# aatifjiwani/lens-flare

Measured on AMD Instinct MI355X. Metric: Mray-surface-intersections/s + frame time, 1080p 256spp double-Gauss, higher is better.
Workload: dtype f32

## Files before the change

lens-flare_amd/csrc/lf_cull_prepass.hip:

```cpp
#include <algorithm>
#include <chrono>
#include <cmath>
#include <cstdio>
#include <cstdlib>
#include <cstring>

#include "lf_internal.h"
#include "lf_march_events.h"
#include "lf_march_common.h"

namespace {

using namespace lfm;

constexpr int kCullSamples = 15;
struct CullLevelArgs {
  int W, H;
  float pitch, half_w, half_h;
  int blocks_x, blocks_y, blk_log2;
  int share_rank, share_n, share_nb;
  int P;
  int P_final;
  int last;
  int n_paths;
// ... 394 lines not shown
__device__ __forceinline__ float ship_extent(const ShipFoot& f, float geo_margin, float nx, float ny) {
  const float e = fabsf(fmaf(f.g1x, nx, f.g1y * ny)) + fabsf(fmaf(f.g2x, nx, f.g2y * ny)) +
                  fabsf(fmaf(f.gxx, nx, f.gxy * ny)) + fabsf(fmaf(f.gyx, nx, f.gyy * ny));
  return fminf(f.ball, fmaf(geo_margin, e, f.slack));
}
__device__ __forceinline__ bool ship_lobe_culls(const ShipFoot& f, float geo_margin, float sx, float sy, float rho) {
  const float ex = sx - f.cx, ey = sy - f.cy;
  const float dist = lf_sqrt(fmaf(ex, ex, ey * ey));
  const float id = dist > 0.0f ? lf_rcp(dist) : 0.0f;
  return dist - kShipLobeK * ship_extent(f, geo_margin, ex * id, ey * id) > rho;
}

template <class A>
__device__ __forceinline__ unsigned ship_lobes_reached(const ShipFoot& f, float geo_margin, unsigned live, const A& a) {
  for (int k = 0; k < a.n_lights; k++)
    if (((live >> k) & 1u) != 0u && ship_lobe_culls(f, geo_margin, a.lsx[k], a.lsy[k], a.lrho[k])) live &= ~(1u << k);
  return live;
}

constexpr unsigned kSlotCulled = 0u, kSlotKept = 1u, kSlotFoot = 2u;
constexpr int kCullMaxLevels = 8;
struct CullCacheOut {
  unsigned* slots;
  float4* foots;
  unsigned* foot_count;
  unsigned foot_cap;
  unsigned n_mine;
};

template <bool BUILD, bool LIGHTS = false>
__device__ __forceinline__ void cull_level_body(const LfLensDev* __restrict__ lens,
                                                    const LfPairsDev* __restrict__ pairs,
                                                    const int* __restrict__ seq_table,
                                                    const LfProgRow* __restrict__ rec_table, const CullLevelArgs& a,
                                                    const unsigned* __restrict__ items,
                                                    const unsigned* __restrict__ counts, unsigned items_stride,
                                                    unsigned* __restrict__ next, unsigned* __restrict__ next_counts,
                                                    unsigned long long* __restrict__ table,
                                                    unsigned long long* __restrict__ stats, const CullCacheOut& co) {
  const int q = blockIdx.y;
  const unsigned PP = (unsigned)(a.P * a.P);
  const unsigned n_blk = (unsigned)(a.blocks_x * a.blocks_y);
  const unsigned n_mine = (n_blk + (unsigned)a.share_n - 1u - (unsigned)a.share_rank) / (unsigned)a.share_n;
  const unsigned n_items = items ? min(counts[q], items_stride) : n_mine * PP;
  const unsigned i = blockIdx.x * blockDim.x + threadIdx.x;
  if ((i & ~63u) >= n_items) return;
  const bool valid = i < n_items;
  const unsigned item = valid ? (items ? items[(size_t)q * items_stride + i]
                                       : ((unsigned)a.share_rank + (unsigned)a.share_n * (i / PP)) * PP + i % PP) : 0u;
  const int blk = (int)(item / PP), cell = (int)(item % PP);
  const int ci = cell % a.P, cj = cell / a.P;
  const int bx = blk % a.blocks_x, by = blk / a.blocks_x;

  const float px0 = (float)(bx << a.blk_log2), px1 = fminf((float)a.W, (float)((bx + 1) << a.blk_log2));
  const float py0 = (float)(by << a.blk_log2), py1 = fminf((float)a.H, (float)((by + 1) << a.blk_log2));
  const float Xc = -((0.5f * (px0 + px1)) - a.half_w) * a.pitch, Yc = -((0.5f * (py0 + py1)) - a.half_h) * a.pitch;
  const float hX = 0.5f * (px1 - px0) * a.pitch, hY = 0.5f * (py1 - py0) * a.pitch;
  const float invP = 1.0f / (float)a.P;

  const int n_ev = pairs->ev_cnt[q];
  const int* const seq = seq_table + pairs->ev_off[q];
  const int lane = (int)(threadIdx.x & 63u);
  constexpr unsigned kAll = (1u << kCullSamples) - 1u;
  const LfProgRow* recs_of[3];
  int j_of[3];
  float ns_of[3];
#pragma unroll
  for (int w = 0; w < 3; w++) {
    const int l = a.lam[w], g = l / a.march_k;
    j_of[w] = l - g * a.march_k;
    recs_of[w] = rec_table + (size_t)g * (size_t)a.prog_recs;
    ns_of[w] = lens->n_start[l];
  }
  Ray r[kCullSamples];
#pragma unroll
  for (int t = 0; t < kCullSamples; t++) {
    float X = Xc, Y = Yc, fu = 0.5f, fv = 0.5f;
    if (t < 9) {
      fu = 0.5f * (float)(t % 3); fv = 0.5f * (float)(t / 3);
      if ((t % 3) != 1 && (t / 3) != 1) { X = Xc + (float)(t % 3 - 1) * hX; Y = Yc + (float)(t / 3 - 1) * hY; }
    }
    else if (t == 9) X = Xc + hX;
    else if (t == 10) X = Xc - hX;
    else if (t == 11) Y = Yc + hY;
    else if (t == 12) Y = Yc - hY;
    const float ns = t == 13 ? ns_of[1] : t == 14 ? ns_of[2] : ns_of[0];
    const float ua = ((float)ci + fu) * invP, ub = ((float)cj + fv) * invP;
    const StartRay s0 = aim_at_pupil(X, Y, fmaf(2.0f, ua, -1.0f), fmaf(2.0f, ub, -1.0f), a.pupil_h, a.vz, a.geom_norm);
    r[t] = Ray{X, Y, 0.0f, 0.0f, s0.dx * ns, s0.dy * ns, s0.dz * ns, 0.0f, 0.0f};
  }
  unsigned live = kAll;
  bool culled = !valid, keep = false;
  int why = 0;
  for (int e = 0; e < n_ev; e++) {
    if (__ballot(!culled && !keep) == 0ull) break;
    const unsigned se = (unsigned)*(const int __attribute__((address_space(4)))*)(seq + e);
    const unsigned kind = se >> 16;
    const LfProgRow wr = load_prec(recs_of[0], se & 0xffffu);
    float cn22_of[3], rn2_of[3], delta_of[3];
#pragma unroll
    for (int w = 0; w < 3; w++) {
      const LfProgRow x = w == 0 ? wr : load_prec(recs_of[w], se & 0xffffu);
      const int j = j_of[w];
      cn22_of[w] = j == 0 ? x.cn22[0] : j == 1 ? x.cn22[1] : x.cn22[2];
      rn2_of[w] = j == 0 ? x.rn2[0] : j == 1 ? x.rn2[1] : x.rn2[2];
      delta_of[w] = j == 0 ? x.delta[0] : j == 1 ? x.delta[1] : x.delta[2];
    }
    const bool stop = (kind & LF_EV_STOP) != 0u;
    unsigned hit = 0u, okm = 0u;
    const unsigned live_before = live;
    float pv[kCullSamples];
#pragma unroll
    for (int t = 0; t < kCullSamples; t++) {
      const int w = t == 13 ? 1 : t == 14 ? 2 : 0;
      bool ok;
      if (stop) {
        const float tt = -(r[t].hz + wr.dzv) * lf_rcp(r[t].dz);
        const float hx = fmaf(tt, r[t].dx, r[t].px), hy = fmaf(tt, r[t].dy, r[t].py);
        r[t].px = hx; r[t].py = hy; r[t].hz = 0.0f;
        ok = hx == hx && hy == hy;
        if (ok) hit |= 1u << t;
        pv[t] = 1.0f;
      } else {
        float disc;
        bool goes_on;
        cull_event(r[t], wr, cn22_of[w], rn2_of[w], delta_of[w], (kind & LF_EV_REFLECT) != 0, (kind & LF_EV_FLAT) != 0, disc, goes_on);
        pv[t] = (kind & LF_EV_REFLECT) ? disc : disc + fminf(0.0f, delta_of[w]);
        const bool reaches = disc >= 0.0f;
        if (reaches) hit |= 1u << t;
        ok = reaches && goes_on;
      }
      if (ok) okm |= 1u << t;
    }
    hit &= live;
    const bool undecided = !culled && !keep;
    const bool all_end = undecided && live_before == kAll && (okm & kAll) == 0u && !stop;
    bool firmly_lost = false;
    if (__ballot(all_end) != 0ull) {
      const float* v = pv;
      const float ga = 0.5f * (v[5] - v[3]), gb = 0.5f * (v[7] - v[1]), gx = 0.5f * (v[9] - v[10]), gy = 0.5f * (v[11] - v[12]);
      const float da = fabsf(0.5f * (v[5] + v[3]) - v[4]), db = fabsf(0.5f * (v[7] + v[1]) - v[4]);
      const float dx = fabsf(0.5f * (v[9] + v[10]) - v[4]), dy = fabsf(0.5f * (v[11] + v[12]) - v[4]);
      const float second = (da + db) + (dx + dy);
      float cross = 0.0f;
#pragma unroll
      for (int t = 0; t < 9; t += 2) {
        if (t == 4) continue;
        const float at = (float)(t % 3 - 1), bt = (float)(t / 3 - 1);
        cross = fmaxf(cross, fabsf((v[t] - v[4]) - fmaf(at, ga + gx, bt * (gb + gy))) - second);
      }
      const float disp = fmaxf(fabsf(v[13] - v[4]), fabsf(v[14] - v[4]));
      const float upper = v[4] + fmaf(a.geo_margin, (fabsf(ga) + fabsf(gb)) + (fabsf(gx) + fabsf(gy)), second + fmaf(2.0f, fmaxf(cross, 0.0f), a.margin * disp));
      firmly_lost = all_end && upper < -1.0e-4f;
    }
    live &= okm;
    const float cx = r[4].px, cy = r[4].py;
    const float cr = lf_sqrt(fmaf(cx, cx, cy * cy));
    const float h = lf_sqrt(wr.h2);
    const bool whole = undecided && hit == kAll;
    if (__ballot(whole && (stop || cr > h)) != 0ull) {
      const ShipFoot f = ship_footprint<false>(r, a.margin, 1e-3f);
      const float icr = cr > 0.0f ? lf_rcp(cr) : 0.0f;
      if (whole && cr - ship_extent(f, a.geo_margin, cx * icr, cy * icr) > h) { culled = true; why = 4; }
      else if (whole && stop) {
        const float s = 0.5f * (float)kCullOcc;
        const float radx = ship_extent(f, a.geo_margin, 1.0f, 0.0f), rady = ship_extent(f, a.geo_margin, 0.0f, 1.0f);
        const int ix0 = max(0, (int)floorf(fmaf(cx - radx, a.inv_stop_h, 1.0f) * s));
        const int ix1 = min(kCullOcc - 1, (int)floorf(fmaf(cx + radx, a.inv_stop_h, 1.0f) * s));
        const int iy0 = max(0, (int)floorf(fmaf(cy - rady, a.inv_stop_h, 1.0f) * s));
        const int iy1 = min(kCullOcc - 1, (int)floorf(fmaf(cy + rady, a.inv_stop_h, 1.0f) * s));
        bool open = false;
        if (ix0 <= ix1) {
          const unsigned span = (ix1 - ix0 >= 31 ? 0xffffffffu : ((2u << (ix1 - ix0)) - 1u)) << ix0;
          for (int iy = iy0; iy <= iy1; iy++) open = open || (a.occ[iy] & span) != 0u;
        }
        if (!open) { culled = true; why = 5; }
      }
    }
    if (undecided && !culled) {
      if (hit == 0u) {
        if (firmly_lost) { culled = true; why = 7; } else { keep = true; why = 2; }
      }
      else if (live == 0u && firmly_lost) { culled = true; why = 7; }
      else if (__popc(live & 0x1ffu) < 3) { keep = true; why = 2; }
    }
  }
  if (!culled && !keep) {
    if (live != kAll) { keep = true; why = 1; }
  }
  if constexpr (BUILD) {
    const bool foot = !culled && !keep;
    const lanemask fm = __ballot(foot);
    unsigned slot = kSlotKept;
    if (fm != 0ull) {
      const ShipFoot f = ship_footprint<true>(r, a.margin, 2e-5f);
      unsigned base = 0u;
      if (lane == (int)__builtin_ctzll(fm)) base = atomicAdd(co.foot_count, (unsigned)__popcll(fm));
      base = __shfl(base, (int)__builtin_ctzll(fm));
      const unsigned at = base + (unsigned)__popcll(fm & ((1ull << lane) - 1ull));
      if (foot && at < co.foot_cap) {
        float4* const o = co.foots + (size_t)at * 3;
        o[0] = make_float4(f.cx, f.cy, f.g1x, f.g1y);
        o[1] = make_float4(f.g2x, f.g2y, f.gxx, f.gxy);
        o[2] = make_float4(f.gyx, f.gyy, f.slack, f.ball);
        slot = kSlotFoot + at;
      }
    }
    if (!culled) co.slots[((size_t)q * co.n_mine + (size_t)(blk / a.share_n)) * PP + (unsigned)cell] = slot;
    keep = !culled;
  } else {
    if (__ballot(!culled && !keep) != 0ull) {
      const ShipFoot f = ship_footprint<true>(r, a.margin, 2e-5f);
      if (!culled && !keep) {
        const bool out = LIGHTS ? ship_lobes_reached(f, a.geo_margin, (1u << a.n_lights) - 1u, a) == 0u
                                : ship_lobe_culls(f, a.geo_margin, a.sx, a.sy, a.rho);
        if (out) { culled = true; why = 6; }
        else { keep = true; why = 3; }
      }
    }
    if (stats && valid && why) atomicAdd(&stats[why], 1ull);
  }
  const bool enabled = valid && keep;
  if (BUILD && a.last) return;
  if (a.last) {
    if (valid && enabled) {
      unsigned long long* row = table + lf_cull_row_of_block(blk, a.share_n, a.share_nb) * (size_t)(a.P * a.P + 1);
      const unsigned long long bit = 1ull << q;
      atomicOr(&row[cell], bit);
    }
    const lanemask em = __ballot(valid && enabled);
    for (lanemask todo = em; todo != 0ull;) {
      const int first = (int)__builtin_ctzll(todo);
      const int b0 = __shfl(blk, first);
      if (lane == first) atomicOr(&table[lf_cull_row_of_block(b0, a.share_n, a.share_nb) * (size_t)(a.P * a.P + 1) + (size_t)(a.P * a.P)], 1ull << q);
      todo &= ~__ballot(blk == b0);
    }
    if (em != 0ull && lane == (int)__builtin_ctzll(em)) atomicAdd(&next_counts[q], (unsigned)__popcll(em));
  } else {
    const lanemask em = __ballot(valid && enabled);
    if (em != 0ull) {
      unsigned base = 0u;
      if (lane == (int)__builtin_ctzll(em)) base = atomicAdd(&next_counts[q], 4u * (unsigned)__popcll(em));
      base = __shfl(base, (int)__builtin_ctzll(em));
      if (valid && enabled) {
        const unsigned at = base + 4u * (unsigned)__popcll(em & ((1ull << lane) - 1ull));
        const unsigned P2 = 2u * (unsigned)a.P;
        unsigned* out = next + (size_t)q * a.list_stride;
        if (at + 3u < a.list_stride) {
#pragma unroll
          for (int c = 0; c < 4; c++)
            out[at + c] = (unsigned)blk * (P2 * P2) + (unsigned)(2 * cj + (c >> 1)) * P2 + (unsigned)(2 * ci + (c & 1));
        }
      }
    }
  }
}

__global__ __launch_bounds__(LF_CULL_WG, LF_CULL_WAVES) void k_cull_level(const LfLensDev* __restrict__ lens,
                                                    const LfPairsDev* __restrict__ pairs,
                                                    const int* __restrict__ seq_table,
                                                    const LfProgRow* __restrict__ rec_table, CullLevelArgs a,
                                                    const unsigned* __restrict__ items,
                                                    const unsigned* __restrict__ counts, unsigned items_stride,
                                                    unsigned* __restrict__ next, unsigned* __restrict__ next_counts,
                                                    unsigned long long* __restrict__ table,
                                                    unsigned long long* __restrict__ stats) {
  cull_level_body<false>(lens, pairs, seq_table, rec_table, a, items, counts, items_stride, next, next_counts, table, stats, CullCacheOut{});
}
__global__ __launch_bounds__(LF_CULL_WG, LF_CULL_WAVES) void k_cull_level_lights(const LfLensDev* __restrict__ lens,
                                                    const LfPairsDev* __restrict__ pairs,
                                                    const int* __restrict__ seq_table,
                                                    const LfProgRow* __restrict__ rec_table, CullLevelArgs a,
                                                    const unsigned* __restrict__ items,
                                                    const unsigned* __restrict__ counts, unsigned items_stride,
                                                    unsigned* __restrict__ next, unsigned* __restrict__ next_counts,
                                                    unsigned long long* __restrict__ table,
                                                    unsigned long long* __restrict__ stats) {
  cull_level_body<false, true>(lens, pairs, seq_table, rec_table, a, items, counts, items_stride, next, next_counts, table, stats, CullCacheOut{});
}
__global__ __launch_bounds__(LF_CULL_WG, LF_CULL_WAVES) void k_cull_level_build(const LfLensDev* __restrict__ lens,
                                                    const LfPairsDev* __restrict__ pairs,
                                                    const int* __restrict__ seq_table,
                                                    const LfProgRow* __restrict__ rec_table, CullLevelArgs a,
                                                    const unsigned* __restrict__ items,
                                                    const unsigned* __restrict__ counts, unsigned items_stride,
                                                    unsigned* __restrict__ next, unsigned* __restrict__ next_counts,
                                                    CullCacheOut co) {
  cull_level_body<true>(lens, pairs, seq_table, rec_table, a, items, counts, items_stride, next, next_counts, nullptr, nullptr, co);
}

struct CullResolveArgs {
  int P_final, n_levels, n_paths, patches;
  int share_rank, share_n, share_nb;
  unsigned n_mine, n_waves;
  float sx, sy, rho, geo_margin;
  const unsigned* slots[kCullMaxLevels];
  const float4* foots[kCullMaxLevels];
  int n_lights;
  float lsx[LF_MAX_LIGHTS], lsy[LF_MAX_LIGHTS], lrho[LF_MAX_LIGHTS];
};
template <bool LIGHTS>
__global__ __launch_bounds__(256) void k_cull_resolve(CullResolveArgs a, unsigned long long* __restrict__ table) {
  const unsigned wave = blockIdx.x * 4u + (threadIdx.x >> 6);
  if (wave >= a.n_waves) return;
  const int lane = (int)(threadIdx.x & 63u);
  const unsigned pp = (unsigned)(a.patches * a.patches);
  const unsigned own = wave / pp, patch = wave % pp;
  const int ci = (int)(patch % (unsigned)a.patches) * 8 + (lane & 7), cj = (int)(patch / (unsigned)a.patches) * 8 + (lane >> 3);
  const bool valid = ci < a.P_final && cj < a.P_final;
  const int blk = a.share_rank + a.share_n * (int)own;
  unsigned long long bits = 0ull;
  for (int q = 0; LIGHTS && q < a.n_paths; q++) {
    unsigned live = valid ? (1u << a.n_lights) - 1u : 0u;
    for (int lv = 0; lv < a.n_levels; lv++) {
      if (__ballot(live != 0u) == 0ull) break;
      const int sh = a.n_levels - 1 - lv;
      const int Pl = a.P_final >> sh;
      if (live != 0u) {
        const unsigned s = a.slots[lv][((size_t)q * a.n_mine + own) * (size_t)(Pl * Pl) + (size_t)((cj >> sh) * Pl + (ci >> sh))];
        if (s == kSlotCulled) live = 0u;
        else if (s >= kSlotFoot) {
          const float4* const p = a.foots[lv] + (size_t)(s - kSlotFoot) * 3;
          const float4 v0 = p[0], v1 = p[1], v2 = p[2];
          const ShipFoot f{v0.x, v0.y, v0.z, v0.w, v1.x, v1.y, v1.z, v1.w, v2.x, v2.y, v2.z, v2.w};
          live = ship_lobes_reached(f, a.geo_margin, live, a);
        }
      }
    }
    if (live != 0u) bits |= 1ull << q;
  }
  for (int q = 0; !LIGHTS && q < a.n_paths; q++) {
    bool alive = valid;
    for (int lv = 0; lv < a.n_levels; lv++) {
      if (__ballot(alive) == 0ull) break;
      const int sh = a.n_levels - 1 - lv;
      const int Pl = a.P_final >> sh;
      if (alive) {
        const unsigned s = a.slots[lv][((size_t)q * a.n_mine + own) * (size_t)(Pl * Pl) + (size_t)((cj >> sh) * Pl + (ci >> sh))];
        if (s == kSlotCulled) alive = false;
        else if (s >= kSlotFoot) {
          const float4* const p = a.foots[lv] + (size_t)(s - kSlotFoot) * 3;
          const float4 v0 = p[0], v1 = p[1], v2 = p[2];
          const ShipFoot f{v0.x, v0.y, v0.z, v0.w, v1.x, v1.y, v1.z, v1.w, v2.x, v2.y, v2.z, v2.w};
          if (ship_lobe_culls(f, a.geo_margin, a.sx, a.sy, a.rho)) alive = false;
        }
      }
    }
    if (alive) bits |= 1ull << q;
  }
  unsigned long long* const row = table + lf_cull_row_of_block(blk, a.share_n, a.share_nb) * (size_t)(a.P_final * a.P_final + 1);
  if (valid) row[cj * a.P_final + ci] = bits;
  unsigned long long any = bits;
  for (int o = 32; o > 0; o >>= 1) any |= __shfl_xor(any, o);
  if (lane == 0 && any != 0ull) atomicOr(&row[a.P_final * a.P_final], any);
}

uint64_t fnv(uint64_t h, const void* data, size_t n) {
  const unsigned char* b = static_cast<const unsigned char*>(data);
  for (size_t i = 0; i < n; i++) { h ^= b[i]; h *= 0x100000001b3ull; }
  return h;
}

}

static int cull_m(const lf_ctx* ctx, int G) {
  (void)ctx;
  int m = 4;
#ifdef LF_EXPERIMENTS
  if (const char* e = std::getenv("LF_CULL_M")) m = std::max(1, std::atoi(e));
#endif
  while (m > 1 && G * m > 128) m >>= 1;
  return m;
}

int lf_cull_reason_of(const lf_ctx* ctx, int G) {
  if (ctx->march_cull == 0) return LF_CULL_OFF;
#ifdef LF_EXPERIMENTS
  if (const char* e = std::getenv("LF_MARCH_CULL")) if (std::atoi(e) == 0) return LF_CULL_OFF;
#endif
  if (ctx->lens.stop < 0) return LF_CULL_NO_STOP;
  if (!ctx->lens_lambda_monotonic) return LF_CULL_DISPERSION;
  if (ctx->pairs.n > 2 * kCullMaxPaths || (ctx->pairs.n > kCullMaxPaths && lf_cull_table_split(ctx))) return LF_CULL_TOO_MANY_PATHS;
  if (G < 1 || G > 64) return LF_CULL_TOO_MANY_SAMPLES;
  if (lf_cull_block_log2(ctx, 1, 1) < 0) return LF_CULL_BLOCK_TOO_LARGE;
  return LF_CULL_APPLIED;
}
bool lf_cull_applies(const lf_ctx* ctx, int G) { return lf_cull_reason_of(ctx, G) == LF_CULL_APPLIED; }

int lf_cull_block_log2(const lf_ctx* ctx, int spp, int n_lambda) {
  const double mm_per_px = (double)ctx->sensor_w_mm / (double)std::max(1, ctx->W);
  int lg = kCullBlockLog2;
  while (lg > 4 && (double)(1 << lg) * mm_per_px > kCullMaxBlockMm) lg--;
  if ((double)(1 << lg) * mm_per_px > kCullMaxBlockMm) return -1;
  if (lg == kCullBlockLog2 && ctx->split.deal != LfSplit::kBlocks && (double)(2 << lg) * mm_per_px <= kCullBigBlockMm && (long long)spp * n_lambda < 768) {
#ifdef LF_EXPERIMENTS
    if (std::getenv("LF_CULL_SMALL_BLOCKS")) return lg;
#endif
    return lg + 1;
  }
  return lg;
}

__global__ void k_cull_popcount(const unsigned long long* __restrict__ table, size_t rows, int cells,
                                unsigned long long* __restrict__ out) {
  const size_t n = rows * (size_t)(cells + 1);
  unsigned long long sum = 0ull;
  for (size_t i = (size_t)blockIdx.x * blockDim.x + threadIdx.x; i < n; i += (size_t)gridDim.x * blockDim.x)
    if ((int)(i % (size_t)(cells + 1)) != cells) sum += (unsigned long long)__popcll(table[i]);
  for (int o = 32; o > 0; o >>= 1) sum += __shfl_xor(sum, o);
  if ((threadIdx.x & 63u) == 0u && sum) atomicAdd(out, sum);
}

constexpr unsigned kDomainAudit = 0x0a0d17c5u;
struct CullAuditArgs {
  int W, H;
  float pitch, half_w, half_h;
  int blocks_x, blocks_y, blk_log2, share_n, share_nb;
  int P, n_paths, n_lambda, march_k, prog_recs;
  float pupil_h, vz, geom_norm, inv_stop_h, lobe_thr;
  int mw, mh;
  uint2 key;
  int density;
  int blk_first, blk_step;
};
template <int VAR>
__device__ __forceinline__ void cull_audit_body(const LfLensDev* __restrict__ lens, const LfPairsDev* __restrict__ pairs,
                                                const int* __restrict__ seq_table, const LfProgRow* __restrict__ rec_table,
                                                const float* __restrict__ mask, const CullAuditArgs& a,
                                                const unsigned long long* __restrict__ table,
                                                unsigned long long* __restrict__ out) {
  constexpr bool LIGHTS = (VAR & kVarLights) != 0;
  const int blk = a.blk_first + (int)blockIdx.y * a.blk_step;
  const int cells = a.P * a.P;
  const int cell = (int)(blockIdx.x * blockDim.x + threadIdx.x);
  if ((cell & ~63) >= cells) return;
  const bool valid = cell < cells;
  const int lane = (int)(threadIdx.x & 63u);
  const unsigned long long* const row = table + lf_cull_row_of_block(blk, a.share_n, a.share_nb) * (size_t)(cells + 1);
  const unsigned long long bits = valid ? row[cell] : ~0ull;
  const int ci = cell % a.P, cj = cell / a.P;
  const int bx = blk % a.blocks_x, by = blk / a.blocks_x;
  const float px0 = (float)(bx << a.blk_log2), px1 = fminf((float)a.W, (float)((bx + 1) << a.blk_log2));
  const float py0 = (float)(by << a.blk_log2), py1 = fminf((float)a.H, (float)((by + 1) << a.blk_log2));
  const float invP = 1.0f / (float)a.P;
  const float sx = lens->sun_dir[0], sy = lens->sun_dir[1], sz = lens->sun_dir[2];
  const float inv_1mc = lens->sun_inv_one_minus_cos, sun_ss = lens->sun_ss;
  unsigned n_rays = 0u, n_lit = 0u;
  for (int q = 0; q < a.n_paths; q++) {
    const bool dropped = valid && ((bits >> q) & 1ull) == 0ull;
    const lanemask todo = __ballot(dropped);
    if (todo == 0ull) continue;
    const int n_ev = pairs->ev_cnt[q];
    const int* const seq = seq_table + pairs->ev_off[q];
    for (int d = 0; d < a.density; d++) {
      const uint4 ru = philox4x32_10(make_uint4((unsigned)blk, blockIdx.x * 4u + (threadIdx.x >> 6), kDomainAudit, (unsigned)(q | (d << 8))), a.key);
      const int l = (int)(__builtin_amdgcn_readfirstlane(ru.x) % (unsigned)a.n_lambda);
      const int g = l / a.march_k, j = l - g * a.march_k;
      const LfProgRow* const recs = rec_table + (size_t)g * (size_t)a.prog_recs;
      const uint4 rnd = philox4x32_10(make_uint4((unsigned)(blk * cells + cell), (unsigned)(q | (d << 8)), kDomainAudit, 1u), a.key);
      const float X = -((px0 + u01(rnd.x) * (px1 - px0)) - a.half_w) * a.pitch;
      const float Y = -((py0 + u01(rnd.y) * (py1 - py0)) - a.half_h) * a.pitch;
      const float ua = ((float)ci + u01(rnd.z)) * invP, ub = ((float)cj + u01(rnd.w)) * invP;
      const StartRay s0 = aim_at_pupil(X, Y, fmaf(2.0f, ua, -1.0f), fmaf(2.0f, ub, -1.0f), a.pupil_h, a.vz, a.geom_norm);
      const float ns = lens->n_start[l];
      Ray r{X, Y, 0.0f, fmaf(X, X, Y * Y), s0.dx * ns, s0.dy * ns, s0.dz * ns, 1.0f, 1.0f};
      lanemask alive = todo;
      n_rays += dropped ? 1u : 0u;
      for (int e = 0; e < n_ev && alive != 0ull; e++) {
        const unsigned se = (unsigned)*(const int __attribute__((address_space(4)))*)(seq + e);
        const LfProgRow wr = load_prec(recs, se & 0xffffu);
        const unsigned kind = se >> 16;
        if (kind & LF_EV_STOP) alive &= stop_event<false>(r, wr.dzv, wr.h2, a.inv_stop_h, mask, a.mw, a.mh);
        else {
          lanemask geom_ok;
          const float cn22 = j == 0 ? wr.cn22[0] : j == 1 ? wr.cn22[1] : wr.cn22[2];
          const float rn2 = j == 0 ? wr.rn2[0] : j == 1 ? wr.rn2[1] : wr.rn2[2];
          const float delta = j == 0 ? wr.delta[0] : j == 1 ? wr.delta[1] : wr.delta[2];
          alive &= surface_event<false>(r, wr.dzv, wr.curv, wr.ch, wr.c2, wr.sc, cn22, rn2, delta, wr.h2, (kind & LF_EV_REFLECT) != 0,
                                        (kind & LF_EV_FLAT) != 0, wr.sgn, geom_ok);
        }
      }
      if (alive == 0ull) continue;
      bool lit;
      if (LIGHTS) {
        lit = false;
        for (int k = 0; k < lens->n_lights; k++) { float qk; lit = light_admits_at<VAR>(lens, k, r.px, r.py, r.hz, r.dx, r.dy, r.dz, qk) || lit; }
        lit = lit && ((alive >> lane) & 1ull) != 0ull;
      } else {
        const float cg = fmaf(r.dx, sx, fmaf(r.dy, sy, r.dz * sz));
        lit = ((alive >> lane) & 1ull) != 0ull && cg > a.lobe_thr && lobe_q(r.dx, r.dy, r.dz, sx, sy, sz, sun_ss, inv_1mc) < 1.0f;
      }
      n_lit += lit ? 1u : 0u;
    }
  }
  unsigned long long v0 = n_rays, v1 = n_lit;
  for (int o = 32; o > 0; o >>= 1) { v0 += __shfl_xor(v0, o); v1 += __shfl_xor(v1, o); }
  if (lane == 0) {
    if (v0) atomicAdd(&out[0], v0);
    if (v1) atomicAdd(&out[1], v1);
  }
}
template <bool LIGHTS>
__global__ __launch_bounds__(256) void k_cull_audit(const LfLensDev* __restrict__ lens, const LfPairsDev* __restrict__ pairs,
                                                    const int* __restrict__ seq_table, const LfProgRow* __restrict__ rec_table,
                                                    const float* __restrict__ mask, CullAuditArgs a,
                                                    const unsigned long long* __restrict__ table,
                                                    unsigned long long* __restrict__ out) {
  cull_audit_body<LIGHTS ? kVarLights : 0>(lens, pairs, seq_table, rec_table, mask, a, table, out);
}
__global__ __launch_bounds__(256) void k_cull_audit_near(const LfLensDev* __restrict__ lens, const LfPairsDev* __restrict__ pairs,
                                                         const int* __restrict__ seq_table, const LfProgRow* __restrict__ rec_table,
                                                         const float* __restrict__ mask, CullAuditArgs a,
                                                         const unsigned long long* __restrict__ table,
                                                         unsigned long long* __restrict__ out) {
  cull_audit_body<kVarLights | kVarNear>(lens, pairs, seq_table, rec_table, mask, a, table, out);
}

lf_status lfk_cull_finish(lf_ctx* ctx, uint64_t hash) {
  if (!ctx->cull_popc_dev) LF_HIP(ctx, hipMalloc((void**)&ctx->cull_popc_dev, 4 * sizeof(unsigned long long)));
  LF_HIP(ctx, hipMemsetAsync(ctx->cull_popc_dev, 0, 4 * sizeof(unsigned long long), ctx->stream));
  const LfCullSlab& slab = ctx->cull_resident;
  const size_t rows = slab.nb > 0 ? (size_t)slab.nb * (size_t)slab.n : (size_t)ctx->cull_bx * ctx->cull_by;
  const int n_blk = ctx->cull_bx * ctx->cull_by;
  const bool own = slab.own_rows_only;
  const int own_n = own ? slab.n : 1, own_rank = own ? slab.rank : 0;
  const int n_own_blk = (n_blk - own_rank + own_n - 1) / own_n;
  const size_t row_entries = (size_t)ctx->cull_cells + 1;
  if (own) hipLaunchKernelGGL(k_cull_popcount, dim3(1024), dim3(256), 0, ctx->stream, ctx->cull_dev + (size_t)own_rank * slab.nb * row_entries,
                              (size_t)n_own_blk, ctx->cull_cells, ctx->cull_popc_dev);
  else hipLaunchKernelGGL(k_cull_popcount, dim3(1024), dim3(256), 0, ctx->stream, ctx->cull_dev, rows, ctx->cull_cells, ctx->cull_popc_dev);
  LF_HIP(ctx, hipGetLastError());
  if (ctx->cull_audit_density > 0) {
    const LfLensDev& L = ctx->lens;
    const LfApertureDev& m = ctx->ap[LF_APERTURE_STARBURST];
    CullAuditArgs a;
    std::memset(&a, 0, sizeof(a));
    a.W = ctx->W; a.H = ctx->H; a.pitch = L.pitch; a.half_w = 0.5f * (float)ctx->W; a.half_h = 0.5f * (float)ctx->H;
    a.blocks_x = ctx->cull_bx; a.blocks_y = ctx->cull_by; a.blk_log2 = ctx->cull_blk_log2;
    a.share_n = slab.n; a.share_nb = slab.nb;
    a.P = ctx->cull_P; a.n_paths = ctx->pairs.n; a.n_lambda = L.n_lambda; a.march_k = ctx->march_k; a.prog_recs = ctx->pairs.prog_recs;
    a.pupil_h = L.pupil_h; a.vz = L.pupil_z - L.z_sensor; a.geom_norm = L.geom_norm; a.inv_stop_h = 1.0f / L.stop_h;
    a.lobe_thr = lf_march_lobe_thr(L);
    a.mw = m.w; a.mh = m.h;
    const float* audit_mask = m.texels;
    if (ctx->mask_filter == LF_MASK_BILINEAR) { audit_mask = m.texels + (size_t)m.w * m.h; a.mw = 2 * m.w; a.mh = 2 * m.h; }
    const uint64_t k = (ctx->cull_audit_seq++) * 0x9e3779b97f4a7c15ull ^ hash;
    a.key = make_uint2((unsigned)k, (unsigned)(k >> 32));
    a.density = ctx->cull_audit_density;
    a.blk_first = own_rank; a.blk_step = own_n;
    const dim3 grid((unsigned)((ctx->cull_cells + 255) / 256), (unsigned)n_own_blk);
    hipEvent_t ev = lf_timing_begin(ctx, LFK_CULL_AUDIT);
    if (lf_has_point_light(L))
      hipLaunchKernelGGL(k_cull_audit_near, grid, dim3(256), 0, ctx->stream, ctx->lens_dev, ctx->pairs_dev,
                         (const int*)(ctx->prog_dev + ctx->prog_seq_off), (const LfProgRow*)(ctx->prog_dev + ctx->prog_rec_off),
                         audit_mask, a, ctx->cull_dev, ctx->cull_popc_dev + 1);
    else if (L.n_lights > 1)
      hipLaunchKernelGGL(k_cull_audit<true>, grid, dim3(256), 0, ctx->stream, ctx->lens_dev, ctx->pairs_dev,
                         (const int*)(ctx->prog_dev + ctx->prog_seq_off), (const LfProgRow*)(ctx->prog_dev + ctx->prog_rec_off),
                         audit_mask, a, ctx->cull_dev, ctx->cull_popc_dev + 1);
    else
    hipLaunchKernelGGL(k_cull_audit<false>, grid, dim3(256), 0, ctx->stream, ctx->lens_dev, ctx->pairs_dev,
                       (const int*)(ctx->prog_dev + ctx->prog_seq_off), (const LfProgRow*)(ctx->prog_dev + ctx->prog_rec_off),
                       audit_mask, a, ctx->cull_dev, ctx->cull_popc_dev + 1);
    lf_timing_end(ctx, LFK_CULL_AUDIT, ev);
    LF_HIP(ctx, hipGetLastError());
  }
  unsigned long long got[4] = {0ull, 0ull, 0ull, 0ull};
  LF_HIP(ctx, hipMemcpyAsync(got, ctx->cull_popc_dev, sizeof(got), hipMemcpyDeviceToHost, ctx->stream));
  LF_HIP(ctx, hipStreamSynchronize(ctx->stream));
  if (ctx->comm_poisoned.load()) return lf_fail(ctx, LF_ERR_STATE, "cull table: the communicator was abandoned while the table was being completed");
  ctx->cull_started_fraction = (double)got[0] / ((double)n_own_blk * (double)ctx->cull_cells * (double)std::max(1, ctx->pairs.n));
  ctx->cull_audit_rays += got[1];
  ctx->cull_audit_lit += got[2];
  ctx->cull_hash = hash;
  ctx->cull_bad_hash = 0;
  if (got[2] != 0ull) {
    ctx->cull_bad_hash = hash;
    ctx->cull_audit_tripped++;
  }
  return LF_OK;
}

static LfCullSlab lf_cull_slab_of(const lf_ctx* ctx, int blk_log2) {
  const LfSplit& s = ctx->split;
  LfCullSlab slab;
  if (s.deal == LfSplit::kBlocks) {
    if (blk_log2 == kDealBlockLog2) { slab.rank = s.rank; slab.n = s.n; slab.own_rows_only = true; }
  } else if (s.table == LfSplit::kComm && ctx->comm_nranks > 1) {
    slab.rank = ctx->comm_rank; slab.n = ctx->comm_nranks;
  } else if (s.table == LfSplit::kHost) {
    slab.rank = s.table_rank; slab.n = s.table_n;
  }
  return slab;
}

static float cull_level_margin(float margin, int P) {
  return margin * (P >= 64 ? 1.0f : P >= 32 ? 1.15f : P >= 16 ? 1.4f : 2.0f);
}

void lf_cull_cache_free(lf_ctx* ctx) {
  LfCullCache& C = ctx->cull_cache;
  if (C.slots) (void)hipFree(C.slots);
  for (float*& f : C.foots) { if (f) (void)hipFree(f); f = nullptr; }
  C.slots = nullptr; C.key = 0; C.reused = false; C.n_levels = 0; C.bytes = 0;
}

static size_t cull_blocks_mine(const CullLevelArgs& a) { return ((size_t)a.blocks_x * a.blocks_y + (size_t)a.share_n - 1 - (size_t)a.share_rank) / (size_t)a.share_n; }

struct CullLevelRun {
  int lv; dim3 grid;
  CullLevelArgs k;
  size_t n_items, total_items;
  const unsigned *items, *items_count; unsigned in_stride;
  unsigned *next, *next_count;
  bool stop = false, synced = false;
};
enum class CullLevelsEnd { kDone, kStopped, kTooLarge };

template <class Kernel, class... Tail>
static void cull_launch_level(lf_ctx* ctx, Kernel kernel, const CullLevelRun& run, Tail... tail) {
  hipLaunchKernelGGL(kernel, run.grid, dim3(LF_CULL_WG), 0, ctx->stream, ctx->lens_dev, ctx->pairs_dev,
                     (const int*)(ctx->prog_dev + ctx->prog_seq_off), (const LfProgRow*)(ctx->prog_dev + ctx->prog_rec_off),
                     run.k, run.items, run.items_count, run.in_stride, run.next, run.next_count, tail...);
}

template <class Launch, class After>
static lf_status cull_run_levels(lf_ctx* ctx, CullLevelArgs a, const int* levels, int n_levels, LfCullLists& lists,
                                 Launch&& launch, After&& after, CullLevelsEnd* end) {
  const float margin = ctx->cull_rules.margin;
  const size_t n_mine = cull_blocks_mine(a);
  unsigned max_items = 0; size_t total_items = 0;
  *end = CullLevelsEnd::kDone;
  for (int lv = 0; lv < n_levels; lv++) {
    a.P = levels[lv]; a.last = lv + 1 == n_levels ? 1 : 0;
    a.margin = cull_level_margin(margin, a.P); a.geo_margin = margin;
    CullLevelRun run; run.lv = lv;
    run.n_items = lv == 0 ? n_mine * (size_t)a.P * a.P : (size_t)max_items;
    run.total_items = lv == 0 ? run.n_items * (size_t)a.n_paths : total_items;
    if (run.n_items == 0) break;
    run.items = lv == 0 ? nullptr : lists.list[(lv - 1) & 1];
    run.items_count = lv == 0 ? nullptr : ctx->cull_counts + (size_t)(lv - 1) * kCullMaxPaths;
    run.in_stride = a.list_stride;
    run.next = nullptr; run.next_count = ctx->cull_counts + (size_t)lv * kCullMaxPaths;
    unsigned out_stride = 0;
    if (!a.last) {
      const size_t need = run.n_items * 4;
      if (need > 0x7fffffffull) { *end = CullLevelsEnd::kTooLarge; return LF_OK; }
      out_stride = (unsigned)need;
      const size_t total = need * (size_t)a.n_paths; const int slot = lv & 1;
      if (total > lists.cap[slot]) {
        LF_HIP(ctx, hipStreamSynchronize(ctx->stream));
// ... 269 lines not shown
```

profiles/microbench/valu_issue.hip:

```cpp
#include <hip/hip_runtime.h>

#include <cstdio>
#include <vector>

template <int MODE>
__global__ __launch_bounds__(256) void k(float* out, int iters, float seed) {
  float a0 = seed + threadIdx.x, a1 = a0 + 1, a2 = a0 + 2, a3 = a0 + 3, a4 = a0 + 4, a5 = a0 + 5,
        a6 = a0 + 6, a7 = a0 + 7;
  const float m = 0.999f, c = 0.001f;
  int sacc = 0;
  typedef float float2v __attribute__((ext_vector_type(2)));
  float2v p0 = {a0, a1}, p1 = {a2, a3}, p2 = {a4, a5}, p3 = {a6, a7}, pm = {m, m}, pc = {c, c};
  for (int i = 0; i < iters; i++) {
#pragma unroll
    for (int u = 0; u < 8; u++) {
      if (MODE == 0) {
        asm volatile("v_fma_f32 %0, %0, %8, %9\n v_fma_f32 %1, %1, %8, %9\n v_fma_f32 %2, %2, %8, %9\n"
                     "v_fma_f32 %3, %3, %8, %9\n v_fma_f32 %4, %4, %8, %9\n v_fma_f32 %5, %5, %8, %9\n"
                     "v_fma_f32 %6, %6, %8, %9\n v_fma_f32 %7, %7, %8, %9\n"
                     : "+v"(a0), "+v"(a1), "+v"(a2), "+v"(a3), "+v"(a4), "+v"(a5), "+v"(a6), "+v"(a7)
                     : "v"(m), "v"(c));
      } else if (MODE == 1) {
        asm volatile("v_fma_f32 %0, %0, %1, %2\n v_fma_f32 %0, %0, %1, %2\n v_fma_f32 %0, %0, %1, %2\n"
                     "v_fma_f32 %0, %0, %1, %2\n v_fma_f32 %0, %0, %1, %2\n v_fma_f32 %0, %0, %1, %2\n"
                     "v_fma_f32 %0, %0, %1, %2\n v_fma_f32 %0, %0, %1, %2\n"
                     : "+v"(a0) : "v"(m), "v"(c));
      } else if (MODE == 2) {
        asm volatile("v_fma_f32 %0, %0, %2, %3\n v_fma_f32 %1, %1, %2, %3\n v_fma_f32 %0, %0, %2, %3\n"
                     "v_fma_f32 %1, %1, %2, %3\n v_fma_f32 %0, %0, %2, %3\n v_fma_f32 %1, %1, %2, %3\n"
                     "v_fma_f32 %0, %0, %2, %3\n v_fma_f32 %1, %1, %2, %3\n"
                     : "+v"(a0), "+v"(a1) : "v"(m), "v"(c));
      } else if (MODE == 3) {
        asm volatile("v_fma_f32 %0, %0, %9, %10\n s_add_u32 %8, %8, 1\n v_fma_f32 %1, %1, %9, %10\n"
                     "v_fma_f32 %2, %2, %9, %10\n s_add_u32 %8, %8, 1\n v_fma_f32 %3, %3, %9, %10\n"
                     "v_fma_f32 %4, %4, %9, %10\n s_add_u32 %8, %8, 1\n v_fma_f32 %5, %5, %9, %10\n"
                     "v_fma_f32 %6, %6, %9, %10\n s_add_u32 %8, %8, 1\n v_fma_f32 %7, %7, %9, %10\n"
                     : "+v"(a0), "+v"(a1), "+v"(a2), "+v"(a3), "+v"(a4), "+v"(a5), "+v"(a6), "+v"(a7),
                       "+s"(sacc)
                     : "v"(m), "v"(c));
      } else if (MODE == 4) {
        asm volatile("v_fma_f32 %0, %0, %2, %3\n s_add_u32 %1, %1, 1\n v_fma_f32 %0, %0, %2, %3\n"
                     "v_fma_f32 %0, %0, %2, %3\n s_add_u32 %1, %1, 1\n v_fma_f32 %0, %0, %2, %3\n"
                     "v_fma_f32 %0, %0, %2, %3\n s_add_u32 %1, %1, 1\n v_fma_f32 %0, %0, %2, %3\n"
                     "v_fma_f32 %0, %0, %2, %3\n s_add_u32 %1, %1, 1\n v_fma_f32 %0, %0, %2, %3\n"
                     : "+v"(a0), "+s"(sacc) : "v"(m), "v"(c));
      } else if (MODE == 5) {
        asm volatile("v_fma_f32 %0, %0, %1, %2\n v_fma_f32 %0, %0, %1, %2\n v_fma_f32 %0, %0, %1, %2\n"
                     "v_sqrt_f32 %0, %0\n v_fma_f32 %0, %0, %1, %2\n v_fma_f32 %0, %0, %1, %2\n"
                     "v_rcp_f32 %0, %0\n v_fma_f32 %0, %0, %1, %2\n"
                     : "+v"(a0) : "v"(m), "v"(c));
      } else if (MODE == 7) {
        asm volatile("v_pk_fma_f32 %0, %0, %4, %5\n v_pk_fma_f32 %1, %1, %4, %5\n v_pk_fma_f32 %2, %2, %4, %5\n"
                     "v_pk_fma_f32 %3, %3, %4, %5\n v_pk_fma_f32 %0, %0, %4, %5\n v_pk_fma_f32 %1, %1, %4, %5\n"
                     "v_pk_fma_f32 %2, %2, %4, %5\n v_pk_fma_f32 %3, %3, %4, %5\n"
                     : "+v"(p0), "+v"(p1), "+v"(p2), "+v"(p3) : "v"(pm), "v"(pc));
      } else if (MODE == 8) {
        asm volatile("v_pk_mul_f32 %0, %0, %4\n v_pk_add_f32 %1, %1, %5\n v_pk_mul_f32 %2, %2, %4\n"
                     "v_pk_add_f32 %3, %3, %5\n v_pk_mul_f32 %0, %0, %4\n v_pk_add_f32 %1, %1, %5\n"
                     "v_pk_mul_f32 %2, %2, %4\n v_pk_add_f32 %3, %3, %5\n"
                     : "+v"(p0), "+v"(p1), "+v"(p2), "+v"(p3) : "v"(pm), "v"(pc));
      } else if (MODE == 9) {
        asm volatile("v_sqrt_f32 %0, %0\n s_nop 0\n v_sqrt_f32 %0, %0\n s_nop 0\n v_sqrt_f32 %0, %0\n s_nop 0\n v_sqrt_f32 %0, %0\n s_nop 0\n"
                     "v_sqrt_f32 %0, %0\n s_nop 0\n v_sqrt_f32 %0, %0\n s_nop 0\n v_sqrt_f32 %0, %0\n s_nop 0\n v_sqrt_f32 %0, %0\n s_nop 0\n"
                     : "+v"(a0));
      } else if (MODE == 10) {
        asm volatile("v_fma_f32 %0, %0, %1, %2\n v_fma_f32 %0, %0, %1, %2\n v_fma_f32 %0, %0, %1, %2\n"
                     "v_sqrt_f32 %0, %0\n s_nop 0\n v_fma_f32 %0, %0, %1, %2\n v_fma_f32 %0, %0, %1, %2\n"
                     "v_fma_f32 %0, %0, %1, %2\n v_fma_f32 %0, %0, %1, %2\n"
                     : "+v"(a0) : "v"(m), "v"(c));
      } else if (MODE == 11) {
        asm volatile("v_fma_f32 %0, %0, %1, %2\n v_sqrt_f32 %0, %0\n s_nop 0\n v_fma_f32 %0, %0, %1, %2\n v_sqrt_f32 %0, %0\n s_nop 0\n"
                     "v_fma_f32 %0, %0, %1, %2\n v_sqrt_f32 %0, %0\n s_nop 0\n v_fma_f32 %0, %0, %1, %2\n v_sqrt_f32 %0, %0\n s_nop 0\n"
                     : "+v"(a0) : "v"(m), "v"(c));
      } else if (MODE == 12) {
        asm volatile("v_fma_f32 %0, %0, %1, %2\n v_fma_f32 %0, %0, %1, %2\n v_fma_f32 %0, %0, %1, %2\n v_fma_f32 %0, %0, %1, %2\n"
                     "v_fma_f32 %0, %0, %1, %2\n v_fma_f32 %0, %0, %1, %2\n v_fma_f32 %0, %0, %1, %2\n v_fma_f32 %0, %0, %1, %2\n"
                     "v_fma_f32 %0, %0, %1, %2\n v_sqrt_f32 %0, %0\n s_nop 0\n v_fma_f32 %0, %0, %1, %2\n v_fma_f32 %0, %0, %1, %2\n"
                     "v_fma_f32 %0, %0, %1, %2\n v_fma_f32 %0, %0, %1, %2\n v_fma_f32 %0, %0, %1, %2\n v_fma_f32 %0, %0, %1, %2\n"
                     "v_sqrt_f32 %0, %0\n s_nop 0\n v_fma_f32 %0, %0, %1, %2\n v_fma_f32 %0, %0, %1, %2\n v_fma_f32 %0, %0, %1, %2\n"
                     "v_fma_f32 %0, %0, %1, %2\n v_fma_f32 %0, %0, %1, %2\n v_fma_f32 %0, %0, %1, %2\n v_fma_f32 %0, %0, %1, %2\n"
                     "v_fma_f32 %0, %0, %1, %2\n v_fma_f32 %0, %0, %1, %2\n v_fma_f32 %0, %0, %1, %2\n"
                     : "+v"(a0) : "v"(m), "v"(c));
      } else if (MODE == 13) {
        asm volatile("v_fma_f32 %0, %0, %4, %5\n v_fma_f32 %0, %0, %4, %5\n v_fma_f32 %0, %0, %4, %5\n v_fma_f32 %0, %0, %4, %5\n v_fma_f32 %0, %0, %4, %5\n v_fma_f32 %0, %0, %4, %5\n v_fma_f32 %0, %0, %4, %5\n v_fma_f32 %0, %0, %4, %5\n v_add_f32 %1, %0, %5\n v_sqrt_f32 %2, %0\n v_sqrt_f32 %3, %1\n s_nop 0\n"
                     "v_fma_f32 %0, %2, %4, %3\n v_fma_f32 %0, %0, %4, %5\n v_fma_f32 %0, %0, %4, %5\n v_fma_f32 %0, %0, %4, %5\n v_fma_f32 %0, %0, %4, %5\n v_fma_f32 %0, %0, %4, %5\n v_fma_f32 %0, %0, %4, %5\n v_fma_f32 %0, %0, %4, %5\n v_fma_f32 %0, %0, %4, %5\n v_fma_f32 %0, %0, %4, %5\n v_fma_f32 %0, %0, %4, %5\n v_fma_f32 %0, %0, %4, %5\n v_fma_f32 %0, %0, %4, %5\n v_fma_f32 %0, %0, %4, %5\n v_fma_f32 %0, %0, %4, %5\n v_fma_f32 %0, %0, %4, %5\n "
                     : "+v"(a0), "+v"(a1), "+v"(a2), "+v"(a3) : "v"(m), "v"(c));
      } else if (MODE == 14) {
        asm volatile("v_fma_f32 %0, %0, %4, %5\n v_fma_f32 %0, %0, %4, %5\n v_fma_f32 %0, %0, %4, %5\n v_fma_f32 %0, %0, %4, %5\n v_fma_f32 %0, %0, %4, %5\n v_fma_f32 %0, %0, %4, %5\n v_fma_f32 %0, %0, %4, %5\n v_fma_f32 %0, %0, %4, %5\n v_fma_f32 %0, %0, %4, %5\n v_sqrt_f32 %2, %0\n v_fma_f32 %1, %1, %4, %5\n v_fma_f32 %1, %1, %4, %5\n v_fma_f32 %1, %1, %4, %5\n v_fma_f32 %0, %2, %4, %5\n v_fma_f32 %0, %0, %4, %5\n v_fma_f32 %0, %0, %4, %5\n "
                     "v_sqrt_f32 %3, %0\n v_fma_f32 %1, %1, %4, %5\n v_fma_f32 %1, %1, %4, %5\n v_fma_f32 %1, %1, %4, %5\n v_fma_f32 %0, %3, %4, %5\n v_fma_f32 %0, %0, %4, %5\n v_fma_f32 %0, %0, %4, %5\n v_fma_f32 %0, %0, %4, %5\n v_fma_f32 %0, %0, %4, %5\n v_fma_f32 %0, %0, %4, %5\n v_fma_f32 %0, %0, %4, %5\n "
                     : "+v"(a0), "+v"(a1), "+v"(a2), "+v"(a3) : "v"(m), "v"(c));
      } else if (MODE == 15) {
        asm volatile("v_fma_f32 %0, %0, %4, %5\n v_fma_f32 %0, %0, %4, %5\n v_fma_f32 %0, %0, %4, %5\n v_fma_f32 %0, %0, %4, %5\n v_fma_f32 %0, %0, %4, %5\n v_fma_f32 %0, %0, %4, %5\n v_fma_f32 %0, %0, %4, %5\n v_fma_f32 %0, %0, %4, %5\n v_add_f32 %1, %0, %5\n v_sqrt_f32 %2, %0\n v_sqrt_f32 %3, %1\n v_fma_f32 %1, %1, %4, %5\n v_fma_f32 %1, %1, %4, %5\n v_fma_f32 %1, %1, %4, %5\n "
                     "v_fma_f32 %0, %2, %4, %3\n v_fma_f32 %0, %0, %4, %5\n v_fma_f32 %0, %0, %4, %5\n v_fma_f32 %0, %0, %4, %5\n v_fma_f32 %0, %0, %4, %5\n v_fma_f32 %0, %0, %4, %5\n v_fma_f32 %0, %0, %4, %5\n v_fma_f32 %0, %0, %4, %5\n v_fma_f32 %0, %0, %4, %5\n v_fma_f32 %0, %0, %4, %5\n v_fma_f32 %0, %0, %4, %5\n v_fma_f32 %0, %0, %4, %5\n v_fma_f32 %0, %0, %4, %5\n "
                     : "+v"(a0), "+v"(a1), "+v"(a2), "+v"(a3) : "v"(m), "v"(c));
      } else if (MODE == 6) {
        asm volatile("v_cmp_gt_f32 vcc, %0, %2\n v_cndmask_b32 %0, %0, %1, vcc\n v_fma_f32 %0, %0, %1, %2\n"
                     "v_cmp_gt_f32 vcc, %0, %2\n v_cndmask_b32 %0, %0, %1, vcc\n v_fma_f32 %0, %0, %1, %2\n"
                     "v_fma_f32 %0, %0, %1, %2\n v_fma_f32 %0, %0, %1, %2\n"
                     : "+v"(a0) : "v"(m), "v"(c) : "vcc");
      }
    }
  }
  out[blockIdx.x * 256 + threadIdx.x] = a0 + a1 + a2 + a3 + a4 + a5 + a6 + a7 + sacc + p0.x + p0.y + p1.x + p1.y + p2.x + p2.y + p3.x + p3.y;
}

template <int MODE>
double run(float* d, int blocks, int iters, int valu_per_iter) {
  hipEvent_t e0, e1;
  hipEventCreate(&e0); hipEventCreate(&e1);
  hipLaunchKernelGGL(k<MODE>, dim3(blocks), dim3(256), 0, 0, d, 100, 1.0f);
  hipDeviceSynchronize();
  hipEventRecord(e0);
  hipLaunchKernelGGL(k<MODE>, dim3(blocks), dim3(256), 0, 0, d, iters, 1.0f);
  hipEventRecord(e1);
  hipEventSynchronize(e1);
  float ms;
  hipEventElapsedTime(&ms, e0, e1);
  double winst = (double)blocks * 4 * iters * 8.0 * valu_per_iter;
  return winst / (ms * 1e-3);
}

int main() {
  float* d;
  hipMalloc(&d, sizeof(float) * 256 * 256 * 16);
  const char* names[] = {"8 independent fma chains", "1 dependent fma chain", "2 interleaved chains",
                         "8 indep fma + 4 SALU per 8", "dependent fma + 4 SALU per 8",
                         "dependent: 6 fma + sqrt + rcp", "dependent: 2x(cmp+cndmask) + 4 fma",
                         "4 indep v_pk_fma_f32 chains", "v_pk_mul/v_pk_add alternating",
                         "dependent: 8 v_sqrt_f32", "dependent: 7 fma + 1 sqrt", "dependent: 4 x (fma, sqrt)",
                         "dependent: event mix 25 fma + 2 sqrt", "event mix, roots adjacent",
                         "event mix, 3 indep fma after each root", "event mix, adjacent + 3 indep"};
  for (int wps : {2, 8}) {
    int blocks = 256 * wps;
    double r[16];
    r[0] = run<0>(d, blocks, 20000, 8);
    r[1] = run<1>(d, blocks, 20000, 8);
    r[2] = run<2>(d, blocks, 20000, 8);
    r[3] = run<3>(d, blocks, 20000, 8);
    r[4] = run<4>(d, blocks, 20000, 8);
    r[5] = run<5>(d, blocks, 20000, 8);
    r[6] = run<6>(d, blocks, 20000, 8);
    r[7] = run<7>(d, blocks, 20000, 8);
    r[8] = run<8>(d, blocks, 20000, 8);
    r[9] = run<9>(d, blocks, 20000, 8);
    r[10] = run<10>(d, blocks, 20000, 8);
    r[11] = run<11>(d, blocks, 20000, 8);
    r[12] = run<12>(d, blocks, 6000, 27);
    r[13] = run<13>(d, blocks, 6000, 27);
    r[14] = run<14>(d, blocks, 6000, 27);
    r[15] = run<15>(d, blocks, 6000, 27);
    for (int i = 0; i < 16; i++)
      if (i != 3 && i != 4) printf("waves/SIMD %d  %-36s %.3e VALU wave-instr/s  (%.2f cyc/instr/SIMD @2.4GHz)\n", wps, names[i],
             r[i], 1024 * 2.4e9 / r[i]);
  }
  return 0;
}
```

Before: 952,000.

## Resolve coarse cull levels cooperatively per patch using shared-memory survivor masks

In the non-lights cull resolve kernel, each wave now evaluates the coarse hierarchy levels once per distinct coarse cell and path, instead of every lane redundantly testing its ancestor cells. Survivors are recorded as per-cell path bitmasks in shared memory with atomicOr, and only the finest level is tested per lane for paths still alive. This removes duplicate slot loads and lobe tests at coarse levels. In exchange it adds block-wide __syncthreads, which forces out-of-range waves to stay resident until the barrier, plus shared atomics. A separate microbenchmark for integer multiply throughput is also added.

```diff
diff --git a/lens-flare_amd/csrc/lf_cull_prepass.hip b/lens-flare_amd/csrc/lf_cull_prepass.hip
--- a/lens-flare_amd/csrc/lf_cull_prepass.hip
+++ b/lens-flare_amd/csrc/lf_cull_prepass.hip
@@ -720,12 +720,13 @@
 template <bool LIGHTS>
 __global__ __launch_bounds__(256) void k_cull_resolve(CullResolveArgs a, unsigned long long* __restrict__ table) {
   const unsigned wave = blockIdx.x * 4u + (threadIdx.x >> 6);
-  if (wave >= a.n_waves) return;
+  const bool in_range = wave < a.n_waves;
+  if (LIGHTS && !in_range) return;
   const int lane = (int)(threadIdx.x & 63u);
   const unsigned pp = (unsigned)(a.patches * a.patches);
   const unsigned own = wave / pp, patch = wave % pp;
   const int ci = (int)(patch % (unsigned)a.patches) * 8 + (lane & 7), cj = (int)(patch / (unsigned)a.patches) * 8 + (lane >> 3);
-  const bool valid = ci < a.P_final && cj < a.P_final;
+  const bool valid = in_range && ci < a.P_final && cj < a.P_final;
   const int blk = a.share_rank + a.share_n * (int)own;
   unsigned long long bits = 0ull;
   for (int q = 0; LIGHTS && q < a.n_paths; q++) {
@@ -747,14 +748,46 @@
     }
     if (live != 0u) bits |= 1ull << q;
   }
-  for (int q = 0; !LIGHTS && q < a.n_paths; q++) {
-    bool alive = valid;
-    for (int lv = 0; lv < a.n_levels; lv++) {
-      if (__ballot(alive) == 0ull) break;
+  if constexpr (!LIGHTS) {
+    __shared__ unsigned long long s_mask[4][kCullMaxLevels][16];
+    unsigned long long (*const mask)[16] = s_mask[threadIdx.x >> 6];
+    const int n_coarse = a.n_levels - 1;
+    for (int i = lane; i < n_coarse * 16; i += 64) mask[i >> 4][i & 15] = 0ull;
+    __syncthreads();
+    const int ci0 = (int)(patch % (unsigned)a.patches) * 8, cj0 = (int)(patch / (unsigned)a.patches) * 8;
+    for (int lv = 0; lv < n_coarse; lv++) {
       const int sh = a.n_levels - 1 - lv;
       const int Pl = a.P_final >> sh;
+      const int side_log2 = sh >= 3 ? 0 : 3 - sh, up_log2 = sh >= 2 ? 0 : 2 - sh;
+      const int n_tests = in_range ? a.n_paths << (2 * side_log2) : 0;
+      for (int t0 = 0; t0 < n_tests; t0 += 64) {
+        const int t = t0 + lane;
+        if (t >= n_tests) continue;
+        const int b = t / a.n_paths, q = t - b * a.n_paths;
+        const int bx = b & ((1 << side_log2) - 1), by = b >> side_log2;
+        const int gx = (ci0 >> sh) + bx, gy = (cj0 >> sh) + by;
+        bool alive = gx < Pl && gy < Pl;
+        if (alive && lv > 0) alive = ((mask[lv - 1][((by >> 1) << up_log2) + (bx >> 1)] >> q) & 1ull) != 0ull;
+        if (!alive) continue;
+        const unsigned s = a.slots[lv][((size_t)q * a.n_mine + own) * (size_t)(Pl * Pl) + (size_t)(gy * Pl + gx)];
+        if (s == kSlotCulled) continue;
+        if (s >= kSlotFoot) {
+          const float4* const p = a.foots[lv] + (size_t)(s - kSlotFoot) * 3;
+          const float4 v0 = p[0], v1 = p[1], v2 = p[2];
+          const ShipFoot f{v0.x, v0.y, v0.z, v0.w, v1.x, v1.y, v1.z, v1.w, v2.x, v2.y, v2.z, v2.w};
+          if (ship_lobe_culls(f, a.geo_margin, a.sx, a.sy, a.rho)) continue;
+        }
+        atomicOr(&mask[lv][b], 1ull << q);
+      }
+      __syncthreads();
+    }
+    const unsigned long long todo = !valid ? 0ull : n_coarse == 0 ? ~0ull : mask[n_coarse - 1][((lane >> 4) << 2) + ((lane & 7) >> 1)];
+    const int lv = n_coarse;
+    for (int q = 0; q < a.n_paths; q++) {
+      bool alive = ((todo >> q) & 1ull) != 0ull;
+      if (__ballot(alive) == 0ull) continue;
       if (alive) {
-        const unsigned s = a.slots[lv][((size_t)q * a.n_mine + own) * (size_t)(Pl * Pl) + (size_t)((cj >> sh) * Pl + (ci >> sh))];
+        const unsigned s = a.slots[lv][((size_t)q * a.n_mine + own) * (size_t)(a.P_final * a.P_final) + (size_t)(cj * a.P_final + ci)];
         if (s == kSlotCulled) alive = false;
         else if (s >= kSlotFoot) {
           const float4* const p = a.foots[lv] + (size_t)(s - kSlotFoot) * 3;
@@ -763,8 +796,9 @@
           if (ship_lobe_culls(f, a.geo_margin, a.sx, a.sy, a.rho)) alive = false;
         }
       }
-    }
-    if (alive) bits |= 1ull << q;
+      if (alive) bits |= 1ull << q;
+    }
+    if (!in_range) return;
   }
   unsigned long long* const row = table + lf_cull_row_of_block(blk, a.share_n, a.share_nb) * (size_t)(a.P_final * a.P_final + 1);
   if (valid) row[cj * a.P_final + ci] = bits;
diff --git a/profiles/microbench/valu_issue.hip b/profiles/microbench/valu_issue.hip
--- a/profiles/microbench/valu_issue.hip
+++ b/profiles/microbench/valu_issue.hip
@@ -102,6 +102,90 @@
     }
   }
   out[blockIdx.x * 256 + threadIdx.x] = a0 + a1 + a2 + a3 + a4 + a5 + a6 + a7 + sacc + p0.x + p0.y + p1.x + p1.y + p2.x + p2.y + p3.x + p3.y;
+}
+
+template <int MODE>
+__global__ __launch_bounds__(256) void ki(unsigned* out, int iters, unsigned seed) {
+  unsigned x = seed + threadIdx.x;
+  uint4 ctr = make_uint4(x, x * 3u + 1u, blockIdx.x, 7u);
+  uint2 key = make_uint2(seed, seed ^ 0x5bd1e995u);
+  unsigned t = 0;
+  const unsigned M0 = 0xD2511F53u, M1 = 0xCD9E8D57u;
+  for (int i = 0; i < iters; i++) {
+#pragma unroll
+    for (int u = 0; u < 8; u++) {
+      if (MODE == 16) {
+        asm volatile("v_mul_lo_u32 %0, %0, %1\n v_mul_lo_u32 %0, %0, %1\n v_mul_lo_u32 %0, %0, %1\n v_mul_lo_u32 %0, %0, %1\n"
+                     "v_mul_lo_u32 %0, %0, %1\n v_mul_lo_u32 %0, %0, %1\n v_mul_lo_u32 %0, %0, %1\n v_mul_lo_u32 %0, %0, %1\n"
+                     : "+v"(x) : "s"(M0));
+      } else if (MODE == 17) {
+        asm volatile("v_mul_hi_u32 %1, %0, %2\n v_mul_lo_u32 %0, %0, %2\n v_mul_hi_u32 %1, %0, %2\n v_mul_lo_u32 %0, %0, %2\n"
+                     "v_mul_hi_u32 %1, %0, %2\n v_mul_lo_u32 %0, %0, %2\n v_mul_hi_u32 %1, %0, %2\n v_mul_lo_u32 %0, %0, %2\n"
+                     : "+v"(x), "+v"(t) : "s"(M0));
+      } else if (MODE == 18) {
+        asm volatile("v_mov_b32 v30, %0\n"
+                     "v_mad_u64_u32 v[30:31], vcc, v30, %1, 0\n v_mad_u64_u32 v[30:31], vcc, v30, %1, 0\n"
+                     "v_mad_u64_u32 v[30:31], vcc, v30, %1, 0\n v_mad_u64_u32 v[30:31], vcc, v30, %1, 0\n"
+                     "v_mad_u64_u32 v[30:31], vcc, v30, %1, 0\n v_mad_u64_u32 v[30:31], vcc, v30, %1, 0\n"
+                     "v_mad_u64_u32 v[30:31], vcc, v30, %1, 0\n v_mad_u64_u32 v[30:31], vcc, v30, %1, 0\n"
+                     "v_xor_b32 %0, v30, v31\n"
+                     : "+v"(x) : "s"(M0) : "v30", "v31", "vcc");
+      } else if (MODE == 19) {
+        const unsigned hi0 = __umulhi(M0, ctr.x), lo0 = M0 * ctr.x;
+        const unsigned hi1 = __umulhi(M1, ctr.z), lo1 = M1 * ctr.z;
+        ctr = make_uint4(hi1 ^ ctr.y ^ key.x, lo1, hi0 ^ ctr.w ^ key.y, lo0);
+        key.x += 0x9E3779B9u; key.y += 0xBB67AE85u;
+      } else if (MODE == 20) {
+        const unsigned long long p0 = (unsigned long long)M0 * ctr.x, p1 = (unsigned long long)M1 * ctr.z;
+        ctr = make_uint4((unsigned)(p1 >> 32) ^ ctr.y ^ key.x, (unsigned)p1, (unsigned)(p0 >> 32) ^ ctr.w ^ key.y, (unsigned)p0);
+        key.x += 0x9E3779B9u; key.y += 0xBB67AE85u;
+      }
+    }
+  }
+  out[blockIdx.x * 256 + threadIdx.x] = x ^ t ^ ctr.x ^ ctr.y ^ ctr.z ^ ctr.w;
+}
+
+template <int MODE>
+double runi(unsigned* d, int blocks, int iters, unsigned* first = nullptr) {
+  hipEvent_t e0, e1;
+  hipEventCreate(&e0); hipEventCreate(&e1);
+  hipLaunchKernelGGL(ki<MODE>, dim3(blocks), dim3(256), 0, 0, d, 100, 1u);
+  hipDeviceSynchronize();
+  if (first) hipMemcpy(first, d, sizeof(unsigned) * 256, hipMemcpyDeviceToHost);
+  hipEventRecord(e0);
+  hipLaunchKernelGGL(ki<MODE>, dim3(blocks), dim3(256), 0, 0, d, iters, 1u);
+  hipEventRecord(e1);
+  hipEventSynchronize(e1);
+  float ms;
+  hipEventElapsedTime(&ms, e0, e1);
+  hipEventDestroy(e0); hipEventDestroy(e1);
+  return (double)blocks * 4 * iters * 8.0 / (ms * 1e-3);
+}
+
+static void integer_multiplies(unsigned* d) {
+  unsigned a[256], b[256];
+  runi<19>(d, 256, 100, a);
+  runi<20>(d, 256, 100, b);
+  bool same = true;
+  for (int i = 0; i < 256; i++) same = same && a[i] == b[i];
+  printf("Philox rounds, pair form vs 64-bit form: %s\n", same ? "same bits" : "DIFFERENT BITS");
+  const char* names[] = {"dependent: v_mul_lo_u32", "v_mul_hi_u32 + v_mul_lo_u32 pair", "dependent: v_mad_u64_u32",
+                         "Philox round, hi/lo pair form", "Philox round, 64-bit product form"};
+  const int per[] = {8, 8, 8, 1, 1};
+  for (int wps : {2, 8}) {
+    const int blocks = 256 * wps;
+    for (int m = 0; m < 5; m++) {
+      double lo = 1e30, hi = 0.0, sum = 0.0;
+      for (int rep = 0; rep < 3; rep++) {
+        const double r = m == 0 ? runi<16>(d, blocks, 4000) : m == 1 ? runi<17>(d, blocks, 4000)
+                       : m == 2 ? runi<18>(d, blocks, 4000) : m == 3 ? runi<19>(d, blocks, 4000) : runi<20>(d, blocks, 4000);
+        const double cyc = 1024 * 2.4e9 / (r * per[m]);
+        lo = cyc < lo ? cyc : lo; hi = cyc > hi ? cyc : hi; sum += cyc;
+      }
+      printf("waves/SIMD %d  %-36s %.2f cyc/%s/SIMD @2.4GHz  (3 runs: %.2f .. %.2f)\n", wps, names[m], sum / 3,
+             m < 3 ? "instr" : "round", lo, hi);
+    }
+  }
 }
 
 template <int MODE>
@@ -153,5 +237,6 @@
       if (i != 3 && i != 4) printf("waves/SIMD %d  %-36s %.3e VALU wave-instr/s  (%.2f cyc/instr/SIMD @2.4GHz)\n", wps, names[i],
              r[i], 1024 * 2.4e9 / r[i]);
   }
+  integer_multiplies((unsigned*)d);
   return 0;
 }
```

Measured after the change: 960,300 (median of 6 runs). About the same (+0.9%).
